# uce/flink-cooccurrence

Hardware: AMD Instinct MI355X
Metric: item-pair co-occurrences counted/sec (node) at 1/2/4/8 GPUs; achieved HBM GB/s (higher is better)
Workload: dtype u32

## Files before the change

flink-cooccurrence_amd/csrc/cooc_sparse.hip:

```cpp
#include "cooc_sparse.h"
#include <algorithm>
#include <cstdio>
#include <string>
#include <type_traits>

namespace cooc {

namespace {

constexpr int kMaxProbe = 64;
constexpr int kSpU = 4;

template <int kWaves>
__device__ inline uint32_t block_excl_scan(uint32_t x, uint32_t *total, uint32_t *s_wtot) {
  const int lane = threadIdx.x & 63, wave = threadIdx.x >> 6;
  const uint32_t inc = wave_incl_scan(x);
  if (lane == 63) s_wtot[wave] = inc;
  __syncthreads();
  uint32_t pre = 0, tot = 0;
#pragma unroll
  for (int w = 0; w < kWaves; w++) {
    const uint32_t v = s_wtot[w];
    pre += w < wave ? v : 0u;
    tot += v;
// ... 208 lines not shown
      uint4 vn[kSpU] = {};
      uint32_t mn = 0;
#pragma unroll
      for (int k = 0; k < kSpU; k++) {
        const uint32_t gk = g + S * (kSpU + k);
        uint32_t mk = 0;
        if (gk < hi) fetch(gk, vn[k], mk);
        mn |= mk << (8 * k);
      }
#pragma unroll
      for (int k = 0; k < kSpU; k++) {
        const uint32_t mk = (m >> (8 * k)) & 255u;
        if (mk) sp_apply_group<Sh, kIds, kMode>(A, L, S_, op, v[k], mk);
#ifdef COOC_SP_STATS
        if (kMode == kWalkHash && k == 0 && !first_seen) {
          first_seen = true;
          if (threadIdx.x == 0) {
            S_.st[54] += STAT_CLOCK() - c_issue;
            S_.st[55] += 1;
          }
        }
#endif
      }
#pragma unroll
      for (int k = 0; k < kSpU; k++) v[k] = vn[k];
      m = mn;
    }
  }
  __syncthreads();
  if (kMode == kWalkHash) STAT_ADD(17, STAT_CLOCK() - c_b1);
  return total;
}

template <class Sh>
__device__ inline uint64_t sp_walk(const SpArgs &A, const SpShared &L, SpStatic &S_, int64_t k0, int64_t k1, int t0,
                                   int t1, bool full, bool bucket, const WalkOp &op) {
  uint64_t walked = 0;
  const int tid = threadIdx.x;
  const bool okt = SP_CHECK(A, t0 >= 0 && t1 <= A.T && t0 <= t1);
  const bool has0 = !bucket && (full || t0 == 0);
  const int ta = full ? 1 : max(t0, 1), tz = full ? A.T : t1;
  const bool has1 = bucket || tz > ta;
  if (bucket) {
    k0 = 0;
    k1 = t1 - t0;
  }
  const uint4 *const ar1 = bucket ? A.scratch + op.sbase : A.tarena;
  const int64_t nsrc1 = bucket ? A.scr_cap : A.n_groups;
  const bool rec = !bucket && A.tbc && (full || (t0 == 0 && !has1));
  constexpr uint32_t kNoList = 0xFFFFFFFFu;
  auto list_of = [&](int64_t b) -> uint32_t {
    if (b + tid >= k1 || !okt) return kNoList;
    const uint32_t u = SP_CHECK(A, b + tid < A.n_contrib) ? A.vals[b + tid] & kListMask : 0u;
    return SP_CHECK(A, u < A.n_users) ? u : 0u;
  };
  auto rec_of = [&](uint32_t u) -> int4 { return u != kNoList ? A.tbc[u] : make_int4(0, 0, 0, 0); };
  int4 rn = make_int4(0, 0, 0, 0);
  uint32_t un = kNoList;
  static_assert(Sh::kDb == Sh::kThreads, "a batch: one contribution per thread");
  if (rec && Sh::kAhead) {
    const uint32_t u0 = list_of(k0);
    un = list_of(k0 + Sh::kDb);
    rn = rec_of(u0);
  }
  for (int64_t b0 = k0; b0 < k1; b0 += Sh::kDb) {
    const int nb = int(min<int64_t>(Sh::kDb, k1 - b0));
    uint32_t s0 = 0, e0 = 0, s1 = 0, e1 = 0;
    STAT_ADD(19, op.mode == kWalkHash && !bucket ? 1 : 0);
    if (bucket) {
      if (tid < nb) {
        s1 = S_.bstart[t0 + tid];
        e1 = s1 + S_.bcur[t0 + tid];
      }
    } else if (rec) {
      if (!Sh::kAhead) rn = rec_of(list_of(b0));
      s0 = uint32_t(rn.x);
      e0 = uint32_t(rn.y);
      if (has1) {
        s1 = uint32_t(rn.z);
        e1 = uint32_t(rn.w);
      }
      if (Sh::kAhead) {
        rn = rec_of(un);
        un = list_of(b0 + 2 * Sh::kDb);
      }
    } else if (tid < nb && okt) {
      const uint32_t u = SP_CHECK(A, b0 + tid < A.n_contrib) ? A.vals[b0 + tid] & kListMask : 0u;
      const int32_t *tbu = A.tb + int64_t(SP_CHECK(A, u < A.n_users) ? u : 0u) * (A.T + 2);
      if (has0) {
        s0 = uint32_t(tbu[0]);
        e0 = uint32_t(tbu[A.T + 1]);
      }
      if (has1) {
        s1 = uint32_t(tbu[ta]);
        e1 = uint32_t(tbu[tz]);
      }
    }
    const unsigned long long c_w0 = STAT_CLOCK();
    if (has0) {
      if (op.mode == kWalkHash)
        walked += sp_walk_batch<Sh, 8, kWalkHash>(A, L, S_, A.tarena0, A.n_groups0, nb, s0, e0, op);
      else
        walked += sp_walk_batch<Sh, 8, kWalkDense>(A, L, S_, A.tarena0, A.n_groups0, nb, s0, e0, op);
    }
    const unsigned long long c_w1 = STAT_CLOCK();
    if (has1) {
      if (op.mode == kWalkHash)
        walked += sp_walk_batch<Sh, 4, kWalkHash>(A, L, S_, ar1, nsrc1, nb, s1, e1, op);
      else if (op.mode == kWalkGather)
        walked += sp_walk_batch<Sh, 4, kWalkGather>(A, L, S_, ar1, nsrc1, nb, s1, e1, op);
      else
        walked += sp_walk_batch<Sh, 4, kWalkDense>(A, L, S_, ar1, nsrc1, nb, s1, e1, op);
    }
#ifdef COOC_SP_STATS
    if (op.split) {
      STAT_ADD(56, c_w1 - c_w0);
      STAT_ADD(57, STAT_CLOCK() - c_w1);
    }
#endif
    if (uni(S_.flag)) break;
  }
  return walked;
}

__device__ inline void sp_global_sync() {
  __builtin_amdgcn_s_waitcnt(0);
  __syncthreads();
  __builtin_amdgcn_fence(__ATOMIC_ACQUIRE, "agent");
}

template <class Sh>
__device__ inline int64_t sp_reserve(const SpArgs &A, SpStatic &S_, int64_t n) {
  const int tid = threadIdx.x;
  if (tid == 0) {
    S_.copy_n = 0;
    if (S_.slab_cur + n > S_.slab_end) {
      const int64_t need = S_.row_n + n;
      const int64_t take = max(A.slab, need + need / 2);
      int64_t b = int64_t(atomicAdd(A.bump, (unsigned long long)take));
      if (b + take > A.cap) {
        atomicOr(reinterpret_cast<unsigned long long *>(&A.tot->err), 4ull);
        S_.pos = -1;
      } else {
        S_.copy_from = S_.row_begin;
        S_.copy_n = S_.row_n;
        S_.row_begin = b;
        S_.slab_cur = b + S_.row_n;
        S_.slab_end = b + take;
        S_.pos = S_.slab_cur;
        S_.slab_cur += n;
      }
    } else {
      S_.pos = S_.slab_cur;
      S_.slab_cur += n;
    }
    if (S_.pos >= 0) S_.row_n += n;
  }
  __syncthreads();
  const int64_t cn = uni(S_.copy_n);
  if (cn > 0) {
    sp_global_sync();
    const int64_t from = S_.copy_from, to = S_.row_begin;
    for (int64_t i = tid; i < cn; i += Sh::kThreads) {
      if (SP_CHECK(A, to + i < A.cap && from + i < A.cap && from >= 0)) {
        A.col_out[to + i] = A.col_out[from + i];
        A.cnt_out[to + i] = A.cnt_out[from + i];
      }
    }
  }
  return uni(S_.pos);
}

template <class Sh>
__device__ inline void sp_dense_compact(const SpArgs &A, const SpShared &L, SpStatic &S_, int32_t w, int32_t c0,
                                        uint64_t &rsum, uint32_t *mdst) {
  constexpr int kPer = Sh::kPer, kStep = 64 * kPer;
  const int tid = threadIdx.x, lane = tid & 63, wave = tid >> 6;
  const unsigned long long c_d0 = STAT_CLOCK();
  uint32_t *row = L.R;
  if (mdst) {
    const int32_t mh = min(w, A.mirror_hi);
    for (int32_t i = tid; i < mh; i += Sh::kThreads) {
      const uint32_t v = Sh::kU16 ? (row[i >> 1] >> ((i & 1) << 4)) & 0xFFFFu : row[i];
      if (!v) continue;
      const int32_t sl = A.mslot[i];
      if (sl >= 0) mdst[int64_t(sl) * A.sstride] = v;
    }
  }
  const int32_t per = ((w + Sh::kWaves - 1) / Sh::kWaves + kStep - 1) & ~(kStep - 1);
  const int32_t lo = min(w, wave * per), hi = min(w, lo + per);
  const uint4 *row4 = reinterpret_cast<const uint4 *>(row);
  auto load = [&](int32_t b, uint32_t v[kPer]) {
    if (b < hi) {
      const uint4 q = row4[b / kPer];
      const uint32_t ww[4] = {q.x, q.y, q.z, q.w};
#pragma unroll
      for (int k = 0; k < kPer; k++) {
        const uint32_t x = Sh::kU16 ? (ww[k >> 1] >> (16 * (k & 1))) & 0xFFFFu : ww[k & 3];
        v[k] = b + k < hi ? x : 0u;
      }
    } else {
#pragma unroll
      for (int k = 0; k < kPer; k++) v[k] = 0u;
    }
  };
  uint32_t cnt = 0;
  for (int32_t b0 = lo; b0 < hi; b0 += kStep) {
    uint32_t v[kPer];
    load(b0 + kPer * lane, v);
#pragma unroll
    for (int k = 0; k < kPer; k++) cnt += v[k] != 0u;
  }
  for (int o = 32; o > 0; o >>= 1) cnt += __shfl_xor(cnt, o, 64);
  if (lane == 0) S_.wtot[wave] = cnt;
  __syncthreads();
  STAT_ADD(48, STAT_CLOCK() - c_d0);
  uint32_t off = 0, tot = 0;
#pragma unroll
  for (int wv = 0; wv < Sh::kWaves; wv++) {
    const uint32_t x = S_.wtot[wv];
    off += wv < wave ? x : 0u;
    tot += x;
  }
  const bool map = A.hot_col != nullptr && c0 == 0;
  constexpr int kW = Sh::kU16 ? 2 : 1, kSub = kPer / kW;
  const int32_t cshift = c0 - (A.hot_col ? kTW : 0);
  uint32_t nxt[kSub][kW];
  auto colq = [&](int32_t b0, bool on) {
#pragma unroll
    for (int k = 0; k < kSub; k++) {
      const int32_t b = b0 + kW * (64 * k + lane);
      if (Sh::kU16) {
        const uint2 t = (on && b < hi) ? *reinterpret_cast<const uint2 *>(A.hot_col + b) : make_uint2(0u, 0u);
        nxt[k][0] = t.x;
        nxt[k][kW - 1] = t.y;
      } else {
        nxt[k][0] = (on && b < hi) ? uint32_t(A.hot_col[b]) : 0u;
      }
    }
  };
  colq(lo, map);
  const int64_t base = sp_reserve<Sh>(A, S_, tot);
  STAT_ADD(49, STAT_CLOCK() - c_d0);
  off = uni(off);
  auto sweep = [&](auto mapped) {
    constexpr bool kMap = decltype(mapped)::value;
    for (int32_t b0 = lo; b0 < hi; b0 += kStep) {
      uint32_t word[kSub], ids[kSub][kW] = {};
#pragma unroll
      for (int k = 0; k < kSub; k++) {
        const int32_t b = b0 + kW * (64 * k + lane);
        word[k] = b < hi ? row[b / kW] : 0u;
      }
      if constexpr (kMap) {
#pragma unroll
        for (int k = 0; k < kSub; k++)
#pragma unroll
          for (int j = 0; j < kW; j++) ids[k][j] = nxt[k][j];
        __builtin_amdgcn_s_waitcnt(0x0F70);
        colq(b0 + kStep, true);
      }
#pragma unroll
      for (int k = 0; k < kSub; k++) {
        const int32_t b = b0 + kW * (64 * k + lane);
        const uint32_t x0 = Sh::kU16 ? word[k] & 0xFFFFu : word[k];
        const uint32_t x1 = (Sh::kU16 && b + 1 < hi) ? word[k] >> 16 : 0u;
        const uint64_t m0 = __ballot(x0 != 0u), m1 = Sh::kU16 ? __ballot(x1 != 0u) : 0ull;
        uint32_t pre = __builtin_amdgcn_mbcnt_hi(uint32_t(m0 >> 32), __builtin_amdgcn_mbcnt_lo(uint32_t(m0), 0u));
        if (Sh::kU16) pre = __builtin_amdgcn_mbcnt_hi(uint32_t(m1 >> 32), __builtin_amdgcn_mbcnt_lo(uint32_t(m1), pre));
        rsum += x0 + x1;
        if (word[k]) {
          const int64_t pos = base + off;
          int32_t *const cp = A.col_out + pos;
          uint32_t *const np = A.cnt_out + pos;
          const uint32_t pre1 = pre + (x0 != 0u);
          if (base >= 0) {
            if (x0 && SP_CHECK(A, pos >= 0 && pos + pre < A.cap)) {
              cp[pre] = kMap ? int32_t(ids[k][0]) : cshift + b;
              np[pre] = x0;
            }
            if (Sh::kU16 && x1 && SP_CHECK(A, pos >= 0 && pos + pre1 < A.cap)) {
              cp[pre1] = kMap ? int32_t(ids[k][kW - 1]) : cshift + b + 1;
              np[pre1] = x1;
            }
          }
          row[b / kW] = 0u;
        }
        off += uint32_t(__popcll(m0)) + uint32_t(__popcll(m1));
      }
    }
  };
  if (map)
    sweep(std::true_type{});
  else
    sweep(std::false_type{});
  STAT_ADD(50, STAT_CLOCK() - c_d0);
  __syncthreads();
  STAT_ADD(51, STAT_CLOCK() - c_d0);
}

template <class Sh>
__device__ inline void sp_hash_compact(const SpArgs &A, const SpShared &L, SpStatic &S_, int32_t H, int32_t c0,
                                       int32_t c1, uint64_t &rsum, uint32_t *mdst) {
  const int tid = threadIdx.x;
  const unsigned long long c_h0 = STAT_CLOCK();
  const uint32_t mhi = mdst ? uint32_t(A.mirror_hi) : 0u;
  uint32_t *keys = L.R, *cnts = L.R + Sh::kHashMax;
  const int per = H / Sh::kThreads;
  const int32_t nL1 = (c1 - c0 + 1023) >> 10;
  uint32_t ek[Sh::kHashMax / Sh::kThreads], ec[Sh::kHashMax / Sh::kThreads], er[Sh::kHashMax / Sh::kThreads];
  (void)per;
#pragma unroll
  for (int q = 0; q < Sh::kHashMax / (4 * Sh::kThreads); q++) {
    const int j = 4 * (tid + q * Sh::kThreads);
    uint4 k4 = make_uint4(0u, 0u, 0u, 0u), v4 = k4;
    if (j < H) {
      k4 = *reinterpret_cast<const uint4 *>(keys + j);
      v4 = *reinterpret_cast<const uint4 *>(cnts + j);
      *reinterpret_cast<uint4 *>(keys + j) = make_uint4(0u, 0u, 0u, 0u);
      *reinterpret_cast<uint4 *>(cnts + j) = make_uint4(0u, 0u, 0u, 0u);
    }
    const uint32_t kk[4] = {k4.x, k4.y, k4.z, k4.w}, vv[4] = {v4.x, v4.y, v4.z, v4.w};
#pragma unroll
    for (int u = 0; u < 4; u++) {
      const int i = 4 * q + u;
      ek[i] = ~0u;
      ec[i] = 0u;
      er[i] = 0u;
      if (kk[u] && vv[u]) {
        const uint32_t col = kk[u] - 1u - uint32_t(c0);
        ek[i] = col;
        ec[i] = vv[u];
        rsum += vv[u];
        if (col < mhi) {
          const int32_t sl = A.mslot[col];
          if (sl >= 0) mdst[int64_t(sl) * A.sstride] = vv[u];
        }
        if (Sh::kRank && !A.any_order) atomicOr(&L.L1[col >> 10], 1u << ((col >> 5) & 31u));
      }
    }
  }
  __syncthreads();
  STAT_ADD(46, STAT_CLOCK() - c_h0);
  if (!Sh::kRank || A.any_order) {
    uint32_t cnt = 0;
#pragma unroll
    for (int i = 0; i < Sh::kHashMax / Sh::kThreads; i++) cnt += ek[i] != ~0u;
    uint32_t ne;
    uint32_t q = block_excl_scan<Sh::kWaves>(cnt, &ne, S_.wtot);
    const unsigned long long c_a1 = STAT_CLOCK();
    STAT_ADD(20, c_a1 - c_h0);
    const int64_t base = sp_reserve<Sh>(A, S_, ne);
    const unsigned long long c_a2 = STAT_CLOCK();
    STAT_ADD(21, c_a2 - c_a1);
    if (base >= 0 && ne <= uint32_t(Sh::kWStage)) {
      uint32_t *sc = keys + Sh::kWStage, *sn = cnts + Sh::kWStage;
#pragma unroll
      for (int i = 0; i < Sh::kHashMax / Sh::kThreads; i++) {
        if (ek[i] == ~0u) continue;
        sc[q] = uint32_t(sp_col(A, uint32_t(c0) + ek[i]));
        sn[q] = ec[i];
        q++;
      }
      __syncthreads();
      const uint32_t head = min(ne, uint32_t((4 - (base & 3)) & 3));
      const uint32_t body = (ne - head) >> 2;
      for (uint32_t j = tid; j < head; j += Sh::kThreads) {
        A.col_out[base + j] = int32_t(sc[j]);
        A.cnt_out[base + j] = sn[j];
      }
      int4 *co4 = reinterpret_cast<int4 *>(A.col_out + base + head);
      uint4 *cn4 = reinterpret_cast<uint4 *>(A.cnt_out + base + head);
      for (uint32_t j = tid; j < body; j += Sh::kThreads) {
        const uint32_t r = head + 4 * j;
        co4[j] = make_int4(int32_t(sc[r]), int32_t(sc[r + 1]), int32_t(sc[r + 2]), int32_t(sc[r + 3]));
        cn4[j] = make_uint4(sn[r], sn[r + 1], sn[r + 2], sn[r + 3]);
      }
      for (uint32_t r = head + 4 * body + tid; r < ne; r += Sh::kThreads) {
        A.col_out[base + r] = int32_t(sc[r]);
        A.cnt_out[base + r] = sn[r];
      }
      __syncthreads();
      for (uint32_t r = tid; r < ne; r += Sh::kThreads) {
        sc[r] = 0u;
        sn[r] = 0u;
      }
    } else if (base >= 0) {
#pragma unroll
      for (int i = 0; i < Sh::kHashMax / Sh::kThreads; i++) {
        if (ek[i] == ~0u) continue;
        if (SP_CHECK(A, base + q < A.cap)) {
          A.col_out[base + q] = sp_col(A, uint32_t(c0) + ek[i]);
          A.cnt_out[base + q] = ec[i];
        }
        q++;
      }
    }
    __syncthreads();
    STAT_ADD(22, STAT_CLOCK() - c_a2);
    STAT_ADD(23, ne);
    return;
  }
  if constexpr (Sh::kRank) {
  uint32_t nblk;
  {
    static_assert(Sh::kL1Words % Sh::kThreads == 0, "L1 words per thread");
    constexpr int kW = Sh::kL1Words / Sh::kThreads;
    uint32_t pc[kW], x = 0;
#pragma unroll
    for (int i = 0; i < kW; i++) {
      pc[i] = kW * tid + i < nL1 ? uint32_t(__popc(L.L1[kW * tid + i])) : 0u;
      x += pc[i];
    }
    const uint32_t p = block_excl_scan<Sh::kWaves>(x, &nblk, S_.wtot);
    uint32_t run = p;
#pragma unroll
    for (int i = 0; i < kW; i++) {
      if (kW * tid + i < nL1) L.L1pre[kW * tid + i] = run;
      run += pc[i];
    }
  }
  __syncthreads();
#pragma unroll
  for (int i = 0; i < Sh::kHashMax / Sh::kThreads; i++) {
    if (ek[i] == ~0u) continue;
    const uint32_t col = ek[i], wd = col >> 10, bit = (col >> 5) & 31u;
    const uint32_t r = L.L1pre[wd] + uint32_t(__popc(L.L1[wd] & ((1u << bit) - 1u)));
    er[i] = r;
    atomicOr(&keys[r], 1u << (col & 31u));
  }
  __syncthreads();
  STAT_ADD(47, STAT_CLOCK() - c_h0);
  const uint32_t pb = (nblk + Sh::kThreads - 1) / Sh::kThreads;
  const uint32_t r0 = min(nblk, uint32_t(tid) * pb), r1 = min(nblk, r0 + pb);
  uint32_t local = 0;
  for (uint32_t r = r0; r < r1; r++) local += uint32_t(__popc(keys[r]));
  uint32_t ne;
  uint32_t run = block_excl_scan<Sh::kWaves>(local, &ne, S_.wtot);
  for (uint32_t r = r0; r < r1; r++) {
    cnts[r] = run;
    run += uint32_t(__popc(keys[r]));
  }
  const unsigned long long c_h1 = STAT_CLOCK();
  STAT_ADD(20, c_h1 - c_h0);
  const int64_t base = sp_reserve<Sh>(A, S_, ne);
  const unsigned long long c_h2 = STAT_CLOCK();
  STAT_ADD(21, c_h2 - c_h1);
  if (base >= 0 && ne <= uint32_t(Sh::kWStage)) {
    uint32_t *sc = keys + Sh::kWStage, *sn = cnts + Sh::kWStage;
    const bool hot0 = A.hot_col && c0 < kTW;
    const uint32_t shift = A.hot_col ? uint32_t(kTW) : 0u;
#pragma unroll
    for (int i = 0; i < Sh::kHashMax / Sh::kThreads; i++) {
      if (ek[i] == ~0u) continue;
      const uint32_t col = ek[i], r = er[i];
      const uint32_t q = cnts[r] + uint32_t(__popc(keys[r] & ((1u << (col & 31u)) - 1u)));
      const uint32_t c = uint32_t(c0) + col;
      sc[q] = hot0 && c < uint32_t(kTW) ? uint32_t(A.hot_col[c]) : c - shift;
      sn[q] = ec[i];
    }
    __syncthreads();
    const uint32_t head = min(ne, uint32_t((4 - (base & 3)) & 3));
    const uint32_t body = (ne - head) >> 2;
    for (uint32_t j = tid; j < head; j += Sh::kThreads) {
      A.col_out[base + j] = int32_t(sc[j]);
      A.cnt_out[base + j] = sn[j];
    }
    int4 *co4 = reinterpret_cast<int4 *>(A.col_out + base + head);
    uint4 *cn4 = reinterpret_cast<uint4 *>(A.cnt_out + base + head);
    for (uint32_t j = tid; j < body; j += Sh::kThreads) {
      const uint32_t q = head + 4 * j;
      co4[j] = make_int4(int32_t(sc[q]), int32_t(sc[q + 1]), int32_t(sc[q + 2]), int32_t(sc[q + 3]));
      cn4[j] = make_uint4(sn[q], sn[q + 1], sn[q + 2], sn[q + 3]);
    }
    for (uint32_t q = head + 4 * body + tid; q < ne; q += Sh::kThreads) {
      A.col_out[base + q] = int32_t(sc[q]);
      A.cnt_out[base + q] = sn[q];
    }
    __syncthreads();
    for (uint32_t q = tid; q < ne; q += Sh::kThreads) {
      sc[q] = 0u;
      sn[q] = 0u;
    }
  } else if (base >= 0) {
#pragma unroll
    for (int i = 0; i < Sh::kHashMax / Sh::kThreads; i++) {
      if (ek[i] == ~0u) continue;
      const uint32_t col = ek[i], r = er[i];
      const int64_t pos = base + cnts[r] + uint32_t(__popc(keys[r] & ((1u << (col & 31u)) - 1u)));
      if (SP_CHECK(A, pos >= 0 && pos < A.cap)) {
        A.col_out[pos] = sp_col(A, uint32_t(c0) + col);
        A.cnt_out[pos] = ec[i];
      }
    }
  }
  __syncthreads();
  STAT_ADD(22, STAT_CLOCK() - c_h2);
  STAT_ADD(23, ne);
  for (uint32_t r = tid; r < nblk; r += Sh::kThreads) {
    keys[r] = 0u;
    cnts[r] = 0u;
  }
  for (int32_t i = tid; i < nL1; i += Sh::kThreads) L.L1[i] = 0u;
  __syncthreads();
  }
}

template <class Sh>
__global__ __launch_bounds__(Sh::kThreads) __attribute__((amdgpu_waves_per_eu(4))) void k_sp_main(SpArgs A) {
  extern __shared__ __attribute__((aligned(16))) uint32_t lds[];
  __shared__ SpStatic S_;
  SpShared L;
  L.R = lds;
  L.L1 = Sh::kRank ? L.R + Sh::kRWords : nullptr;
  L.L1pre = Sh::kRank ? L.L1 + Sh::kL1Words : nullptr;
  L.gb = reinterpret_cast<int32_t *>(L.R + Sh::kRWords + Sh::kBmWords);
  L.info = reinterpret_cast<uint32_t *>(L.gb + Sh::kDb);
  L.vst = L.info + Sh::kDb;
  L.qstart = reinterpret_cast<int32_t *>(L.vst + Sh::kDb + 4);
  const int tid = threadIdx.x;
  for (int32_t i = tid; i < Sh::kRWords + (Sh::kRank ? Sh::kL1Words : 0); i += Sh::kThreads) L.R[i] = 0u;
  if (tid == 0) {
    S_.slab_cur = S_.slab_end = 0;
    S_.flag = 0u;
  }
  const int64_t n_work = A.q_end - A.q_begin;
#ifdef COOC_SP_STATS
  if (threadIdx.x < 64) S_.st[threadIdx.x] = 0ull;
  const unsigned long long t_start = STAT_CLOCK();
#endif
  if (tid == 0) S_.work = atomicAdd(A.qctr, 1);
  __syncthreads();
  uint64_t rsum = 0;
  for (;;) {
    const int32_t w = uni(S_.work);
    if (w >= n_work) break;
    uint32_t next = 0;
    if (tid == 0) next = atomicAdd(A.qctr, 1);
    const SpWork it = A.queue[A.q_begin + w];
    const int32_t a = it.row;
    const int32_t ra = sp_rank(A, a);
    const bool split = it.kind == -2;
    const int64_t k0 = it.k0, k1 = it.k1;
    int t = 0;
    const int t_end = (split && A.mirror_hi > 0) ? 1 : A.T;
    uint32_t *const mdst = (!split && A.mirror_hi > 0 && ra >= kTW) ? A.staging + ra : nullptr;
    const uint64_t st = it.st, dn = it.dn, hz0 = it.hz[0], hz1 = it.hz[1];
    bool gather = A.scr_cap > 0 && it.gslot >= 0;
    if (!split && tid == 0) {
      const int64_t e = it.est;
      S_.own = 0u;
      if (e > A.slab / 4 && e + e / 8 > S_.slab_end - S_.slab_cur) {
        const int64_t take = e + e / 8 + 1024;
        const int64_t b = int64_t(atomicAdd(A.bump, (unsigned long long)take));
        if (b + take <= A.cap) {
          S_.saved_cur = S_.slab_cur;
          S_.saved_end = S_.slab_end;
          S_.own = 1u;
          S_.slab_cur = b;
          S_.slab_end = b + take;
        }
      }
      S_.row_begin = S_.slab_cur;
      S_.row_n = 0;
      S_.rsum = 0ull;
    }
    const int64_t rs_expect = (!split && tid == 0) ? A.rowsum[a] : 0;
    if (gather && tid < 64) {
      const float Wi = float(A.epre[k1] - A.epre[k0]);
      uint32_t cap = 0;
      if (tid >= 1 && tid < A.T) cap = (uint32_t(1.1f * Wi * A.gmass[tid]) + 64u + 3u) & ~3u;
      const uint32_t inc = wave_incl_scan(cap);
      if (tid < A.T) {
        S_.bstart[tid] = inc - cap;
        S_.bcur[tid] = 0u;
      }
      if (tid == A.T - 1) S_.bstart[A.T] = inc;
    }
    __syncthreads();
    gather = gather && uni(S_.bstart[A.T]) <= uint32_t(A.scr_cap) * 4u;
    const int dense_until = split ? t_end : -1;
    int32_t H = 0;
    bool deferred = !split && A.sort_all;
    if (deferred) t = t_end;
    while (t < t_end) {
      const bool dense = t < dense_until || ((dn >> t) & 1ull);
      int t1 = t + 1;
      if (!dense) {
        const uint64_t rest = t + 1 < 64 ? st >> (t + 1) : 0ull;
        t1 = rest ? min(t_end, t + __ffsll((long long)rest)) : t_end;
        if (H == 0) H = min(Sh::kHashMax, kHashMin << (((t < 32 ? hz0 : hz1) >> (2 * (t & 31))) & 3u));
      }
      const int32_t c0 = t * kTW, c1 = min(A.M, t1 * kTW);
      WalkOp op;
      op.mode = dense ? kWalkDense : kWalkHash;
      const uint32_t lg = dense ? 0u : 31u - uint32_t(__clz(uint32_t(H)));
      op.hshift = 32u - lg;
      op.hmask = uint32_t(H) - 1u;
      if (tid == 0) {
        S_.flag = 0u;
      }
      __syncthreads();
      const unsigned long long c_walk = STAT_CLOCK();
      op.sbase = int64_t(blockIdx.x) * A.scr_cap;
#ifdef COOC_SP_STATS
      op.split = split;
#endif
      const bool gwalk = gather && t == 0;
      const bool bucket = gather && !gwalk &&
                          !(uint64_t(uni(int64_t(S_.ovf))) & (((t1 < 64 ? (1ull << t1) : 0ull) - 1ull) & ~((1ull << t) - 1ull)));
      if (gwalk) op.mode = kWalkGather;
      const uint64_t walked = sp_walk<Sh>(A, L, S_, k0, k1, gwalk ? 0 : t, gwalk ? A.T : t1,
                                          gwalk || (!split && t == 0 && t1 == A.T), bucket, op);
      if (gwalk) {
        if (tid < 64) {
          const bool o = tid >= 1 && tid < A.T && S_.bcur[tid] > S_.bstart[tid + 1] - S_.bstart[tid];
          const uint64_t m = __ballot(o);
          if (tid == 0) S_.ovf = m;
        }
        sp_global_sync();
      }
      if (bucket && split) STAT_ADD(58, STAT_CLOCK() - c_walk);
      const unsigned long long c_walked = STAT_CLOCK();
      STAT_ADD(split ? 4 : dense ? 0 : 1, c_walked - c_walk);
#ifdef COOC_SP_STATS
      const int hcls = (!split && t == 0 && t1 == t_end) ? 0 : (gather && t > 0) ? 1 : 2;
      if (!dense && !split) {
        STAT_ADD(28 + 6 * hcls, 1);
        STAT_ADD(29 + 6 * hcls, c_walked - c_walk);
        STAT_ADD(31 + 6 * hcls, walked);
        STAT_ADD(33 + 6 * hcls, k1 - k0);
      }
#endif
      STAT_ADD(dense ? 9 : 10, walked);
      STAT_ADD(dense ? 5 : 6, 1);
      if (!dense && uni(S_.flag)) {
        STAT_ADD(7, 1);
        for (int32_t j = tid; j < H; j += Sh::kThreads) {
          L.R[j] = 0u;
          L.R[Sh::kHashMax + j] = 0u;
        }
        deferred = true;
        __syncthreads();
        break;
      }
      const uint32_t self = uint32_t(A.spre ? A.spre[k1] - A.spre[k0] : k1 - k0);
      if (split) {
        uint32_t *dst = A.staging + int64_t(A.split_slot[a]) * A.sstride + c0;
        if (!Sh::kU16) {
          for (int32_t i = tid; i < c1 - c0; i += Sh::kThreads) {
            const uint32_t v = L.R[i];
            if (v) {
              atomicAdd(dst + i, v);
              L.R[i] = 0u;
            }
          }
        }
        __syncthreads();
        STAT_ADD(26, STAT_CLOCK() - c_walked);
      } else if (dense) {
        if (tid == 0 && ra >= c0 && ra < c1) {
          const uint32_t o = uint32_t(ra - c0);
          if (Sh::kU16)
            L.R[o >> 1] -= self << ((o & 1u) << 4);
          else
            L.R[o] -= self;
        }
        __syncthreads();
        sp_dense_compact<Sh>(A, L, S_, c1 - c0, c0, rsum, c0 == 0 ? mdst : nullptr);
        STAT_ADD(2, STAT_CLOCK() - c_walked);
      } else {
        if (tid == 0 && ra >= c0 && ra < c1) {
          uint32_t h = (uint32_t(ra) * 0x9E3779B1u) >> op.hshift;
          for (int p = 0; p < H; p++) {
            if (L.R[h] == uint32_t(ra) + 1u) {
              L.R[Sh::kHashMax + h] -= self;
              break;
            }
            h = (h + 1u) & op.hmask;
          }
        }
        __syncthreads();
        sp_hash_compact<Sh>(A, L, S_, H, c0, c1, rsum, c0 == 0 ? mdst : nullptr);
        STAT_ADD(3, STAT_CLOCK() - c_walked);
#ifdef COOC_SP_STATS
        STAT_ADD(30 + 6 * hcls, STAT_CLOCK() - c_walked);
        STAT_ADD(32 + 6 * hcls, uni(S_.row_n));
#endif
        STAT_ADD(14, H);
      }
      t = t1;
      H = 0;
    }
    STAT_ADD(split ? 12 : 11, 1);
    if (deferred) {
      STAT_ADD(8, 1);
      rsum = 0;
      if (tid == 0) {
        A.deferred[atomicAdd(reinterpret_cast<unsigned long long *>(&A.tot->n_deferred), 1ull)] = a;
        if (!S_.own) S_.slab_cur = S_.row_begin;
        S_.row_n = 0;
// ... 445 lines not shown
```

Before: 366.8 billion.

## Replace LDS-staged hash compaction with wave-ballot direct scattered writes

The any-order compaction path now counts surviving entries per wave with ballots and stores the per-wave totals before the existing barrier, so the separate block scan and its extra barrier go away. Each wave computes its own offsets with mbcnt and writes column/count pairs directly to global memory. This replaces staging in shared memory, vectorized uint4 stores, and the re-zeroing pass. Hot-column remapping is also hoisted into registers ahead of the reserve call. The cost is narrower, less coalesced global stores in exchange for fewer barriers and less LDS traffic.

```diff
diff --git a/flink-cooccurrence_amd/csrc/cooc_sparse.hip b/flink-cooccurrence_amd/csrc/cooc_sparse.hip
--- a/flink-cooccurrence_amd/csrc/cooc_sparse.hip
+++ b/flink-cooccurrence_amd/csrc/cooc_sparse.hip
@@ -534,7 +534,8 @@
 template <class Sh>
 __device__ inline void sp_hash_compact(const SpArgs &A, const SpShared &L, SpStatic &S_, int32_t H, int32_t c0,
                                        int32_t c1, uint64_t &rsum, uint32_t *mdst) {
-  const int tid = threadIdx.x;
+  int tid = threadIdx.x;
+  asm volatile("" : "+v"(tid));
   const unsigned long long c_h0 = STAT_CLOCK();
   const uint32_t mhi = mdst ? uint32_t(A.mirror_hi) : 0u;
   uint32_t *keys = L.R, *cnts = L.R + Sh::kHashMax;
@@ -572,63 +573,70 @@
       }
     }
   }
+  const bool any = !Sh::kRank || A.any_order;
+  constexpr int kE = Sh::kHashMax / Sh::kThreads;
+  if (any) {
+    uint32_t wc = 0;
+#pragma unroll
+    for (int i = 0; i < kE; i++) wc += uint32_t(__popcll(__ballot(ek[i] != ~0u)));
+    if ((tid & 63) == 0) S_.wtot[tid >> 6] = wc;
+  }
   __syncthreads();
   STAT_ADD(46, STAT_CLOCK() - c_h0);
-  if (!Sh::kRank || A.any_order) {
-    uint32_t cnt = 0;
-#pragma unroll
-    for (int i = 0; i < Sh::kHashMax / Sh::kThreads; i++) cnt += ek[i] != ~0u;
-    uint32_t ne;
-    uint32_t q = block_excl_scan<Sh::kWaves>(cnt, &ne, S_.wtot);
+  if (any) {
+    const int wave = tid >> 6;
+    uint32_t off = 0, ne = 0;
+#pragma unroll
+    for (int wv = 0; wv < Sh::kWaves; wv++) {
+      const uint32_t x = S_.wtot[wv];
+      off += wv < wave ? x : 0u;
+      ne += x;
+    }
+    ne = uni(ne);
+    const bool map = A.hot_col != nullptr && c0 == 0;
+    if (map) {
+#pragma unroll
+      for (int i = 0; i < kE; i++) {
+        const uint32_t c = ek[i];
+        if (c != ~0u) ek[i] = c < uint32_t(kTW) ? uint32_t(A.hot_col[c]) : c - uint32_t(kTW);
+      }
+    }
     const unsigned long long c_a1 = STAT_CLOCK();
     STAT_ADD(20, c_a1 - c_h0);
     const int64_t base = sp_reserve<Sh>(A, S_, ne);
     const unsigned long long c_a2 = STAT_CLOCK();
     STAT_ADD(21, c_a2 - c_a1);
-    if (base >= 0 && ne <= uint32_t(Sh::kWStage)) {
-      uint32_t *sc = keys + Sh::kWStage, *sn = cnts + Sh::kWStage;
-#pragma unroll
-      for (int i = 0; i < Sh::kHashMax / Sh::kThreads; i++) {
-        if (ek[i] == ~0u) continue;
-        sc[q] = uint32_t(sp_col(A, uint32_t(c0) + ek[i]));
-        sn[q] = ec[i];
-        q++;
-      }
-      __syncthreads();
-      const uint32_t head = min(ne, uint32_t((4 - (base & 3)) & 3));
-      const uint32_t body = (ne - head) >> 2;
-      for (uint32_t j = tid; j < head; j += Sh::kThreads) {
-        A.col_out[base + j] = int32_t(sc[j]);
-        A.cnt_out[base + j] = sn[j];
-      }
-      int4 *co4 = reinterpret_cast<int4 *>(A.col_out + base + head);
-      uint4 *cn4 = reinterpret_cast<uint4 *>(A.cnt_out + base + head);
-      for (uint32_t j = tid; j < body; j += Sh::kThreads) {
-        const uint32_t r = head + 4 * j;
-        co4[j] = make_int4(int32_t(sc[r]), int32_t(sc[r + 1]), int32_t(sc[r + 2]), int32_t(sc[r + 3]));
-        cn4[j] = make_uint4(sn[r], sn[r + 1], sn[r + 2], sn[r + 3]);
-      }
-      for (uint32_t r = head + 4 * body + tid; r < ne; r += Sh::kThreads) {
-        A.col_out[base + r] = int32_t(sc[r]);
-        A.cnt_out[base + r] = sn[r];
-      }
-      __syncthreads();
-      for (uint32_t r = tid; r < ne; r += Sh::kThreads) {
-        sc[r] = 0u;
-        sn[r] = 0u;
-      }
-    } else if (base >= 0) {
-#pragma unroll
-      for (int i = 0; i < Sh::kHashMax / Sh::kThreads; i++) {
-        if (ek[i] == ~0u) continue;
-        if (SP_CHECK(A, base + q < A.cap)) {
-          A.col_out[base + q] = sp_col(A, uint32_t(c0) + ek[i]);
-          A.cnt_out[base + q] = ec[i];
+    off = uni(off);
+    const uint32_t cshift = uint32_t(c0) - (A.hot_col ? uint32_t(kTW) : 0u);
+    using gi32 = __attribute__((address_space(1))) int32_t;
+    using gu32 = __attribute__((address_space(1))) uint32_t;
+    gi32 *co = (gi32 *)(A.col_out + max<int64_t>(base, int64_t(0)));
+    gu32 *cn = (gu32 *)(A.cnt_out + max<int64_t>(base, int64_t(0)));
+    asm volatile("" : "+s"(co), "+s"(cn));
+    auto write = [&](auto mapped) {
+      constexpr bool kMap = decltype(mapped)::value;
+      if constexpr (kMap) __builtin_amdgcn_s_waitcnt(0x0F70);
+#pragma unroll
+      for (int i = 0; i < kE; i++) {
+        const bool on = ek[i] != ~0u;
+        const uint64_t m = __ballot(on);
+        const uint32_t pre = __builtin_amdgcn_mbcnt_hi(uint32_t(m >> 32), __builtin_amdgcn_mbcnt_lo(uint32_t(m), 0u));
+        const int64_t pos = base + off;
+        (void)pos;
+        if (on && SP_CHECK(A, pos >= 0 && pos + pre < A.cap)) {
+          (co + off)[pre] = int32_t(kMap ? ek[i] : cshift + ek[i]);
+          (cn + off)[pre] = ec[i];
         }
-        q++;
-      }
-    }
-    __syncthreads();
+        off += uint32_t(__popcll(m));
+        __builtin_amdgcn_sched_barrier(0);
+      }
+    };
+    if (base >= 0) {
+      if (map)
+        write(std::true_type{});
+      else
+        write(std::false_type{});
+    }
     STAT_ADD(22, STAT_CLOCK() - c_a2);
     STAT_ADD(23, ne);
     return;
```

Measured after the change: 372.6 billion (median of 6 runs). 1.6% higher.
